# zlib-ng/minizip-ng

Measured on NVIDIA H100. Metric: deflate_l1_crc32_input_throughput, higher is better.
Workload: dtype u8

## Files before the change

minizip-ng_b200/csrc/deflate_kernel.cuh:

```cuda
#ifndef MZ_DEFLATE_KERNEL_CUH
#define MZ_DEFLATE_KERNEL_CUH

#include "mzcuda_common.cuh"

namespace mzc {

constexpr int DF_THREADS = 512;
constexpr int DF_WARPS = DF_THREADS / 32;
constexpr int DF_CHUNK_MAX = 65536;
constexpr int DF_UNIT = 32768;
constexpr int DF_SB = DF_UNIT;
constexpr int DF_SPAN = 8;
constexpr int DF_BATCH = DF_THREADS * DF_SPAN;
constexpr int DF_NBATCH = DF_UNIT / DF_BATCH;
constexpr int DF_MINMATCH = 4;
constexpr int DF_LOCKLEN = 8;
constexpr int DF_HASH_BITS = 13;
constexpr int DF_HASH_ENTRIES = 1 << DF_HASH_BITS;
constexpr int DF_STAGE_WORDS = DF_UNIT / 4 + 64;
constexpr int DF_HDR_WORDS = 96;

constexpr uint32_t DF_FLAG_FINAL = 1u;
constexpr uint32_t DF_FLAG_DICT = 2u;

constexpr int DF_OFF_IN = 0;
constexpr int DF_OFF_HASH = DF_OFF_IN + DF_UNIT + 64;
constexpr int DF_OFF_STAGE = DF_OFF_HASH;
constexpr int DF_OFF_REC = DF_OFF_HASH + DF_STAGE_WORDS * 4;
constexpr int DF_OFF_SPN = DF_OFF_REC + DF_NBATCH * DF_THREADS * 8;
constexpr int DF_SPAN_BYTES = DF_NBATCH * DF_THREADS * 10;
constexpr int DF_OFF_HIST = DF_OFF_REC + DF_SPAN_BYTES;
constexpr int DF_OFF_HIST2 = DF_OFF_HIST + (288 + 32) * 4;
constexpr int DF_OFF_CODE = DF_OFF_HIST2 + 256 * 4;
constexpr int DF_OFF_LENS = DF_OFF_CODE + (288 + 32) * 4;
constexpr int DF_OFF_BITS = DF_OFF_LENS + (288 + 32);
constexpr int DF_OFF_SCAN = DF_OFF_BITS + (288 + 32);
constexpr int DF_OFF_BB = DF_OFF_SCAN + 256 * 4;
constexpr int DF_OFF_MISC = DF_OFF_BB + 512 * 4;
constexpr int DF_OFF_SINK = DF_OFF_MISC + 32 * 4 + 16;
constexpr int DF_OFF_LSYM = DF_OFF_SINK + 32 * 4;
constexpr int DF_SMEM_BYTES = DF_OFF_LSYM + 256 * 2;
constexpr uint32_t DF_ZERO_SYM = 286;
static_assert(DF_HASH_ENTRIES * 4 <= DF_STAGE_WORDS * 4, "hash fits the staging region");
constexpr int DFH_PREV = 32768;
constexpr int DFH_HASH_BITS = 14;
constexpr int DFH_OFF_HASH = (DF_SMEM_BYTES + 15) & ~15;
constexpr int DFH_SMEM_BYTES = DFH_PREV + DFH_OFF_HASH + (4 << DFH_HASH_BITS);
static_assert(DFH_SMEM_BYTES <= 227 * 1024, "shared memory budget of the history variant");
static_assert(DF_SMEM_BYTES <= 113 * 1024, "shared memory budget for two CTAs per SM");

enum { MISC_CHUNK = 3, MISC_CARRY = 8  };

struct DeflateParams {
    const uint8_t *in;
    const uint64_t *in_off;
    const uint32_t *in_len;
    const uint8_t *flags;
    uint64_t total_len;
    uint32_t chunk_size;
    uint32_t nchunks;
    uint32_t last_flags;
    int32_t level;
    uint8_t *out;
    uint64_t slot_stride;
    uint32_t *out_len;
    uint32_t *work_counter;
};

__host__ __device__ inline uint64_t deflate_slot_bound(uint32_t chunk_size) {
    return (((uint64_t)chunk_size + 12ull * ((chunk_size + DF_SB - 1) / DF_SB + 1) + 64 + 15) & ~15ull);
}

__device__ __forceinline__ void length_symbol(uint32_t len, uint32_t &sym, uint32_t &ebits, uint32_t &eval) {
    const uint32_t l = len - 3;
    const uint32_t msb = 31u - (uint32_t)__clz((int)(l | 4u));
    uint32_t e = msb - 2;
    uint32_t sy = 4 * (e + 1) + ((l >> e) & 3u);
    uint32_t ev = l & ((1u << e) - 1u);
    sy = l < 8 ? l : sy;
    const bool top = len == 258;
    sym = top ? 28u : sy;
    ebits = top ? 0u : e;
    eval = top ? 0u : ev;
}
__device__ __forceinline__ void dist_symbol0(uint32_t d, uint32_t &sym, uint32_t &ebits) {
    uint32_t m = 31u - (uint32_t)__clz((int)(d | 1u));
    ebits = m > 0 ? m - 1 : 0u;
    sym = 2 * m + ((d >> ebits) & 1u);
}
__device__ __forceinline__ uint32_t len_extra_bits(uint32_t lsym) { return (lsym < 8 || lsym >= 28) ? 0u : (lsym >> 2) - 1; }
__device__ __forceinline__ uint32_t dist_extra_bits(uint32_t dsym) { return dsym < 4 ? 0u : (dsym >> 1) - 1; }

__device__ __forceinline__ uint32_t stage_word(uint32_t base, uint32_t pos, uint32_t k4) { return base + __umulhi(pos, 1u << 27) * k4; }

__device__ __forceinline__ void stage_put(uint32_t *stage, uint32_t pos, uint32_t v, uint32_t n) {
    if (n == 0) return;
    if (n < 32) v &= (1u << n) - 1;
    uint32_t w = pos >> 5, s = pos & 31;
    atomicOr(&stage[w], v << s);
    if (s + n > 32) atomicOr(&stage[w + 1], v >> (32 - s));
}

__device__ __forceinline__ void stage_or(const Smem &sm, uint32_t pos, uint32_t v, uint32_t n) {
    const uint32_t sh = pos & 31u, wa = DF_OFF_STAGE + ((pos >> 5) << 2);
    sm.red_or32(wa, v << sh);
    if (sh + n > 32) sm.red_or32(wa + 4, v >> (32 - sh));
}

struct BitWriter {
    Smem sm;
    uint64_t acc;
    uint32_t nb, wa;
    __device__ __forceinline__ void init(const Smem &s, uint32_t bitoff) {
        sm = s; wa = DF_OFF_STAGE + (bitoff >> 5) * 4; nb = bitoff & 31; acc = 0;
    }
    __device__ __forceinline__ void put(uint32_t v, uint32_t n) {
        acc |= (uint64_t)v << nb;
        nb += n;
        if (nb >= 32) {
            sm.red_or32(wa, (uint32_t)acc);
            acc >>= 32; nb -= 32; wa += 4;
        }
    }
    __device__ __forceinline__ uint32_t bitpos() const { return ((wa - (uint32_t)DF_OFF_STAGE) << 3) + nb; }
    __device__ __forceinline__ void finish() {
        if (nb > 0) sm.red_or32(wa, (uint32_t)acc);
        if (nb > 32) sm.red_or32(wa + 4, (uint32_t)(acc >> 32));
    }
};

__device__ inline uint32_t block_excl_sum(uint32_t v, uint32_t *scan, uint32_t &total) {
    uint32_t incl = warp_incl_sum(v);
    if (lane_id() == 31) scan[warp_id()] = incl;
    __syncthreads();
    if (warp_id() == 0) {
        uint32_t w = lane_id() < (unsigned)DF_WARPS ? scan[lane_id()] : 0u;
        uint32_t wi = warp_incl_sum(w);
        scan[32 + lane_id()] = wi - w;
        if (lane_id() == 31) scan[31] = wi;
    }
    __syncthreads();
    uint32_t res = scan[32 + warp_id()] + incl - v;
    total = scan[31];
    __syncthreads();
    return res;
}

constexpr int DF_BB_THREADS = 320;
enum { BB_STAT = 0 , BB_KRAFT = 8 , BB_K = 72 ,
       BB_NEXT = 104 , BB_SLACK = 136 , BB_CNTW = 144 ,
       BB_NZ = 464 , BB_ST = 474 ,
       BB_HSUM = 484 , BB_HDRBITS = 494  };

constexpr uint64_t CL_LENS = 0x12ddad91b725bb4ull;
constexpr uint64_t CL_CODE_LO = 0x840013930ef3c6ull, CL_CODE_HI = 0xd5c7fdf6cb149ull;
constexpr uint64_t CL_ORDER57 = 0x1b6d6db248db92dull;
__device__ __forceinline__ uint32_t cl_len(uint32_t s) { return (uint32_t)(CL_LENS >> (3 * s)) & 7u; }
__device__ __forceinline__ uint32_t cl_code(uint32_t s) {
    return s < 10 ? (uint32_t)(CL_CODE_LO >> (6 * s)) & 63u : (uint32_t)(CL_CODE_HI >> (6 * (s - 10))) & 63u;
}

__device__ __forceinline__ void bb_count_lengths(uint32_t *cntw_row, uint32_t L, unsigned lane, unsigned &m) {
    if (lane < 16) cntw_row[lane] = 0;
    __syncwarp();
    m = __match_any_sync(MZ_FULL_MASK, L);
    if (L > 0 && lane == (unsigned)(__ffs((int)m) - 1)) cntw_row[L] = (uint32_t)__popc(m);
    __syncwarp();
}

__device__ inline void block_build_codes(const uint32_t *hist_ll, const uint32_t *hist_lit2, const uint32_t *hist_d, uint8_t *lens_ll, uint8_t *lens_d,
                                         uint32_t *code_ll, uint32_t *code_d, uint8_t *bits_ll, uint8_t *bits_d, uint32_t *bb,
                                         uint32_t *stage, uint32_t hdrpos, uint32_t bfinal) {
    const uint32_t tid = threadIdx.x;
    const unsigned lane = lane_id(), w = warp_id();
    const int a = tid < 288 ? 0 : (tid < 320 ? 1 : 2);
    const uint32_t sym = a == 0 ? tid : tid - 288;
    const uint32_t nsym = a == 0 ? 286u : 30u;
    const int M = 15;
    const uint32_t one = 1u << M;
    const uint32_t w0 = a == 0 ? 0u : 9u;
    uint32_t c = (a < 2 && sym < nsym) ? (a == 0 ? hist_ll[sym] + (sym < 256 ? hist_lit2[sym] : 0u) : hist_d[sym]) : 0u;

    if (tid < 144) bb[tid] = (tid == BB_STAT + 2 || tid == BB_STAT + 6) ? 0xffffffffu : 0u;
    bar_sync(1, DF_BB_THREADS);
    if (a < 2) {
        uint32_t used_w = __reduce_add_sync(MZ_FULL_MASK, c ? 1u : 0u);
        uint32_t tot_w = __reduce_add_sync(MZ_FULL_MASK, c);
        uint32_t first_w = __reduce_min_sync(MZ_FULL_MASK, c ? sym : 0xffffffffu);
        if (lane == 0) {
            atomicAdd(&bb[BB_STAT + a * 4 + 0], used_w);
            atomicAdd(&bb[BB_STAT + a * 4 + 1], tot_w);
            atomicMin(&bb[BB_STAT + a * 4 + 2], first_w);
        }
    }
    bar_sync(1, DF_BB_THREADS);
    float ideal = 0.f;
    if (a < 2) {
        uint32_t used = bb[BB_STAT + a * 4 + 0], total = bb[BB_STAT + a * 4 + 1], fu = bb[BB_STAT + a * 4 + 2];
        if (used < 2) {
            uint32_t d0 = used == 0 ? 0u : (fu == 0 ? 1u : 0u);
            uint32_t d1 = used == 0 ? 1u : d0;
            if ((sym == d0 || sym == d1) && c == 0) c = 1;
            total += 2 - used;
        }
        if (c) ideal = __log2f((float)total) - __log2f((float)c);
    }
    float lo = -3.0f, step = 0.25f;
    uint32_t slack[2] = {0, 0};
    for (int sweep = 0; sweep < 2; sweep++) {
        if (a < 2) {
#pragma unroll
            for (int cnd = 0; cnd < 16; cnd++) {
                uint32_t kr = 0;
                if (c) {
                    int l = (int)ceilf(ideal - (lo + step * (float)cnd));
                    l = l < 1 ? 1 : (l > M ? M : l);
                    kr = 1u << (M - l);
                }
                kr = __reduce_add_sync(MZ_FULL_MASK, kr);
                if (lane == 0) atomicAdd(&bb[BB_KRAFT + sweep * 32 + a * 16 + cnd], kr);
            }
        }
        bar_sync(1, DF_BB_THREADS);
        float lo_a = lo;
        for (int aa = 0; aa < 2; aa++) {
            int best = 0;
            for (int cnd = 1; cnd < 16; cnd++)
                if (bb[BB_KRAFT + sweep * 32 + aa * 16 + cnd] <= one) best = cnd;
            slack[aa] = one - bb[BB_KRAFT + sweep * 32 + aa * 16 + best];
            if (aa == a) lo_a = lo + step * (float)best;
        }
        lo = lo_a;
        step *= 0.0625f;
    }
    uint32_t L = 0;
    if (c) {
        int l = (int)ceilf(ideal - lo);
        L = (uint32_t)(l < 1 ? 1 : (l > M ? M : l));
    }
    unsigned m = 0;
    int buf = 0;
    for (int pass = 0; pass < 40; pass++) {
        if (slack[0] == 0 && slack[1] == 0) break;
        uint32_t *cntw = bb + BB_CNTW + buf * 160;
        if (a < 2) bb_count_lengths(cntw + w * 16, L, lane, m);
        bar_sync(1, DF_BB_THREADS);
        if (w == 0 || w == 9) {
            const int aa = w == 0 ? 0 : 1;
            const uint32_t wa = aa == 0 ? 0u : 9u, wb = aa == 0 ? 9u : 10u;
            uint32_t tot = 0;
            if (lane >= 2 && lane <= (unsigned)M)
                for (uint32_t ww = wa; ww < wb; ww++) tot += cntw[ww * 16 + lane];
            uint32_t sl = slack[aa], myk = 0;
            for (int len = 2; len <= M; len++) {
                uint32_t t = __shfl_sync(MZ_FULL_MASK, tot, len);
                uint32_t can = sl >> (M - len);
                uint32_t k = t < can ? t : can;
                if (lane == (unsigned)len) myk = k;
                sl -= k << (M - len);
            }
            if (lane >= 2 && lane <= (unsigned)M) bb[BB_K + aa * 16 + lane] = myk;
            if (lane == 0) bb[BB_SLACK + aa] = sl;
        }
        bar_sync(1, DF_BB_THREADS);
        if (a < 2 && L >= 2) {
            uint32_t rank = (uint32_t)__popc(m & ((1u << lane) - 1));
            for (uint32_t ww = w0; ww < w; ww++) rank += cntw[ww * 16 + L];
            if (rank < bb[BB_K + a * 16 + L]) L -= 1;
        }
        slack[0] = bb[BB_SLACK + 0];
        slack[1] = bb[BB_SLACK + 1];
        buf ^= 1;
    }
    uint32_t *cntw = bb + BB_CNTW + buf * 160;
    if (a < 2) bb_count_lengths(cntw + w * 16, L, lane, m);
    bar_sync(1, DF_BB_THREADS);
    if (w == 0 || w == 9) {
        const int aa = w == 0 ? 0 : 1;
        const uint32_t wa = aa == 0 ? 0u : 9u, wb = aa == 0 ? 9u : 10u;
        uint32_t tot = 0;
        if (lane >= 1 && lane <= (unsigned)M)
            for (uint32_t ww = wa; ww < wb; ww++) tot += cntw[ww * 16 + lane];
        uint32_t code = 0, prev = 0, mycode = 0;
        for (int len = 1; len <= M; len++) {
            code = (code + prev) << 1;
            if (lane == (unsigned)len) mycode = code;
            prev = __shfl_sync(MZ_FULL_MASK, tot, len);
        }
        if (lane >= 1 && lane <= (unsigned)M) bb[BB_NEXT + aa * 16 + lane] = mycode;
    }
    bar_sync(1, DF_BB_THREADS);
    if (a < 2) {
        uint32_t cw = 0;
        if (L) {
            uint32_t rank = (uint32_t)__popc(m & ((1u << lane) - 1));
            for (uint32_t ww = w0; ww < w; ww++) rank += cntw[ww * 16 + L];
            uint32_t code = bb[BB_NEXT + a * 16 + L] + rank;
            cw = (__brev(code) >> (32 - L)) | (L << 16);
        }
        if (a == 0) {
            const uint32_t eb = sym >= 257 ? len_extra_bits(sym - 257) : 0u;
            lens_ll[sym] = (uint8_t)L;
            code_ll[sym] = cw | (eb << 20);
            bits_ll[sym] = (uint8_t)(L + eb);
        } else {
            lens_d[sym] = (uint8_t)L;
            code_d[sym] = cw;
            bits_d[sym] = (uint8_t)(L + dist_extra_bits(sym));
        }
    }
    const unsigned nz = __ballot_sync(MZ_FULL_MASK, L != 0);
    if (lane == 0) bb[BB_NZ + w] = nz;
    bar_sync(1, DF_BB_THREADS);
    const uint32_t hlit = 256u + 32u - (uint32_t)__clz((int)bb[BB_NZ + 8]);
    const uint32_t hdw = bb[BB_NZ + 9];
    const uint32_t hdist = hdw ? 32u - (uint32_t)__clz((int)hdw) : 1u;
    const uint32_t nlen = a == 0 ? hlit : hdist;
    const bool valid = sym < nlen;
    const uint32_t prevL = sym == 0 ? 0xffu : (a == 0 ? lens_ll[sym - 1] : lens_d[sym - 1]);
    const unsigned st = __ballot_sync(MZ_FULL_MASK, (valid && prevL != L) || sym == nlen);
    if (lane == 0) bb[BB_ST + w] = st;
    bar_sync(1, DF_BB_THREADS);
    uint32_t nb = 0, val = 0;
    if (valid) {
        uint32_t m = st & (0xffffffffu >> (31u - lane)), ww = w;
        while (m == 0) m = bb[BB_ST + --ww];
        const uint32_t s0 = (ww - w0) * 32u + 31u - (uint32_t)__clz((int)m);
        m = lane == 31 ? 0u : st & (0xfffffffeu << lane);
        ww = w;
        while (m == 0) m = bb[BB_ST + ++ww];
        const uint32_t e0 = (ww - w0) * 32u + (uint32_t)__ffs((int)m) - 1u;
        const uint32_t k = sym - s0, R = e0 - s0;
        uint32_t cs = L, ev = 0, eb = 0;
        bool tok = true;
        if (L == 0) {
            const uint32_t full = (R / 138u) * 138u, rem = R - full;
            if (k < full) { tok = k % 138u == 0; cs = 18; ev = 127; eb = 7; }
            else if (rem >= 11) { tok = k == full; cs = 18; ev = rem - 11; eb = 7; }
            else if (rem >= 3) { tok = k == full; cs = 17; ev = rem - 3; eb = 3; }
        } else if (k > 0) {
            const uint32_t k1 = k - 1, rest = R - 1, full = (rest / 6u) * 6u, rem = rest - full;
            if (k1 < full) { tok = k1 % 6u == 0; cs = 16; ev = 3; eb = 2; }
            else if (rem >= 3) { tok = k1 == full; cs = 16; ev = rem - 3; eb = 2; }
        }
        if (tok) {
            const uint32_t cl = cl_len(cs);
            nb = cl + eb;
            val = cl_code(cs) | (ev << cl);
        }
    }
    const uint32_t incl = warp_incl_sum(nb);
    if (lane == 31) bb[BB_HSUM + w] = incl;
    bar_sync(1, DF_BB_THREADS);
    uint32_t off = incl - nb, total = 0;
    for (uint32_t ww = 0; ww < 10; ww++) {
        const uint32_t t = bb[BB_HSUM + ww];
        off += ww < w ? t : 0u;
        total += t;
    }
    if (nb) stage_put(stage, hdrpos + 17 + 57 + off, val, nb);
    if (tid == 0) {
        stage_put(stage, hdrpos, bfinal | (2u << 1) | ((hlit - 257u) << 3) | ((hdist - 1u) << 8) | (15u << 13), 17);
        bb[BB_HDRBITS] = 17 + 57 + total;
    }
    if (tid == 32) stage_put(stage, hdrpos + 17, (uint32_t)CL_ORDER57, 32);
    if (tid == 64) stage_put(stage, hdrpos + 17 + 32, (uint32_t)(CL_ORDER57 >> 32), 25);
}

__device__ __forceinline__ uint32_t extend_match8(const Smem &sm, uint32_t c, uint32_t q, uint32_t maxlen) {
    uint32_t len = 8;
    while (len < maxlen) {
        uint32_t x = sm.ld32u(DF_OFF_IN, q + len) ^ sm.ld32u(DF_OFF_IN, c + len);
        if (x) {
            len += (uint32_t)(__ffs((int)x) - 1) >> 3;
            break;
        }
        len += 4;
    }
    return len < maxlen ? len : maxlen;
}

__device__ __forceinline__ uint32_t opaque4() { return blockDim.x / (uint32_t)(DF_THREADS / 4); }

template <bool HIST>
__device__ __forceinline__ uint32_t hash_addr(uint32_t v, uint32_t k4) {
    return (HIST ? DFH_OFF_HASH : DF_OFF_HASH) + __umulhi(v * 2654435761u, 1u << (HIST ? DFH_HASH_BITS : DF_HASH_BITS)) * k4;
}

__device__ __forceinline__ uint32_t rec_len(uint32_t r) { uint32_t l = (r >> 3) & 255u; return l ? l + 3 : 0u; }

__device__ __forceinline__ uint32_t fin_len(uint32_t m) { return ((m >> 4) & 255u) + 3u; }
__device__ __forceinline__ uint32_t fin_dist(uint32_t m) { return ((m >> 12) & 0x7fffu) + 1u; }
template <bool ONEM>
__device__ __forceinline__ void span_classify(const Smem &sm, uint32_t A, uint32_t B, uint32_t q0, uint32_t cover, uint32_t &F, uint32_t &MA,
                                              uint32_t &MB) {
    const uint32_t lit = (A >> 26) | ((B >> 26) << 6);
    const uint32_t crel = cover > q0 ? cover - q0 : 0u;
    const uint32_t cr8 = crel < 8 ? crel : 8u;
    uint32_t ex = 0;
    MA = MB = 0;
#pragma unroll
    for (int r = 0; r < (ONEM ? 1 : 2); r++) {
        const uint32_t R = r == 0 ? A : B;
        const uint32_t j = R & 7u, end = j + rec_len(R);
        const uint32_t s = j > crel ? j : crel;
        const uint32_t Lf = (end > s ? end : s) - s;
        const uint32_t P = (s < 8u ? s : 8u) & 7u;
        const uint32_t M = Lf >= 3 ? (((Lf << 4) + (0x80000000u - (3u << 4))) | P | ((R << 1) & (0x7fffu << 12))) : 0u;
        if (r == 0) MA = M;
        else MB = M;
        ex = Lf - 1u < 2u ? Lf : ex;
    }
    F = ((lit >> cr8) << cr8) | (ex << 8);
    if (ex) {
        const uint32_t p = DF_OFF_IN + q0 + crel;
        F |= sm.ld8(p) << 16;
        if (ex == 2) F |= sm.ld8(p + 1) << 24;
    }
}

__device__ __forceinline__ uint32_t match_symbols(const Smem &sm, uint32_t M) {
    uint32_t ds, db;
    const uint32_t lsv = sm.ld16(DF_OFF_LSYM + ((M >> 3) & 0x1feu));
    const uint32_t d = fin_dist(M) - 1;
    dist_symbol0(d, ds, db);
    sm.red_add32(DF_OFF_HIST + (257u + (lsv & 31u)) * 4, 1u);
    sm.red_add32(DF_OFF_HIST + (288u + ds) * 4, 1u);
    return 0x80000000u | ((M & 7u) << 28) | ((d & ((1u << db) - 1u)) << 15) | (ds << 10) | lsv;
}
__device__ __forceinline__ uint32_t match_bits(const Smem &sm, uint32_t M) {
    const uint32_t n = sm.ld8(DF_OFF_BITS + 257u + (M & 31u)) + sm.ld8(DF_OFF_BITS + 288u + ((M >> 10) & 31u));
    return M ? n : 0u;
}
__device__ __forceinline__ void put_match_bits(const Smem &sm, uint32_t pos, uint32_t M) {
    const uint32_t cwl = sm.ld32(DF_OFF_CODE + (257u + (M & 31u)) * 4);
    const uint32_t cwd = sm.ld32(DF_OFF_CODE + (288u + ((M >> 10) & 31u)) * 4);
    const uint32_t cl = (cwl >> 16) & 15u, cd = (cwd >> 16) & 15u;
    const uint32_t v1 = (cwl & 0x7fffu) | (((M >> 5) & 31u) << cl);
    const uint32_t n1 = cl + ((cwl >> 20) & 15u);
    const uint32_t v2 = (cwd & 0x7fffu) | (((M >> 15) & 0x1fffu) << cd);
    const uint64_t V = (uint64_t)v1 | ((uint64_t)v2 << n1);
    const uint32_t lo = (uint32_t)V, hi = (uint32_t)(V >> 32);
    const uint32_t wa = stage_word(DF_OFF_STAGE, pos, opaque4());
    const uint32_t w0 = __funnelshift_l(0u, lo, pos), w1 = __funnelshift_l(lo, hi, pos), w2 = __funnelshift_l(hi, 0u, pos);
    sm.red_or32(wa, w0);
    sm.red_or32(wa + 4, w1);
    if (w2) sm.red_or32(wa + 8, w2);
}

__device__ __forceinline__ uint32_t nth_parked(const uint32_t (&bm)[DF_NBATCH], uint32_t k, uint32_t warp) {
    uint32_t r = k, word = 0, bsel = 0;
    bool found = false;
#pragma unroll
    for (int b = 0; b < DF_NBATCH; b++) {
        const uint32_t c = (uint32_t)__popc(bm[b]);
        const bool here = !found && r < c;
        word = here ? bm[b] : word;
        bsel = here ? (uint32_t)b : bsel;
        found = found || here;
        r -= found ? 0u : c;
    }
    uint32_t base = 0;
#pragma unroll
    for (int st = 16; st; st >>= 1) {
        const uint32_t c = (uint32_t)__popc((word >> base) & ((1u << st) - 1u));
        const bool up = r >= c;
        r -= up ? c : 0u;
        base += up ? (uint32_t)st : 0u;
    }
    return found ? bsel * (uint32_t)DF_THREADS + warp * 32u + base : 0xffffffffu;
}

enum { DF_PH_LOAD, DF_PH_PARSE, DF_PH_M0, DF_PH_COVER, DF_PH_T_M1, DF_PH_D, DF_PH_E_SCAN, DF_PH_F_M3, DF_PH_FLUSH, DF_PH_UNITS, DF_PH_COLS };
constexpr int DF_PH_ROWS = 1024;
#if defined(MZ_DF_PHASES) && !defined(MZ_EMU)
__device__ unsigned long long g_df_phases[DF_PH_ROWS][DF_PH_COLS];
#define DF_PHASE_BEGIN(t) unsigned long long t = clock64()
#define DF_PHASE(t, ph)                                                                        \
    do {                                                                                       \
        if (threadIdx.x == 0 && blockIdx.x < (unsigned)DF_PH_ROWS) {                           \
            const unsigned long long now_ = clock64();                                         \
            atomicAdd(&g_df_phases[blockIdx.x][ph], now_ - (t));                               \
            if ((ph) == DF_PH_LOAD) atomicAdd(&g_df_phases[blockIdx.x][DF_PH_UNITS], 1ull);   \
            (t) = now_;                                                                        \
        }                                                                                      \
    } while (0)
#else
#define DF_PHASE_BEGIN(t)
#define DF_PHASE(t, ph)
#endif

template <int STRIDE, bool LAZY, bool HIST = false>
__global__ void __launch_bounds__(DF_THREADS, HIST ? 1 : 2) deflate_chunks_kernel(DeflateParams P) {
    MZ_DYN_SMEM(smem_raw);
    uint8_t *const smem = smem_raw + (HIST ? DFH_PREV : 0);
    constexpr uint32_t CUR = HIST ? (uint32_t)DFH_PREV : 0u;
    uint8_t *s_in = smem + DF_OFF_IN;
    uint32_t *s_stage = (uint32_t *)(smem + DF_OFF_STAGE);
    uint32_t *s_hist_ll = (uint32_t *)(smem + DF_OFF_HIST);
    uint32_t *s_hist_d = s_hist_ll + 288;
    uint32_t *s_code_ll = (uint32_t *)(smem + DF_OFF_CODE);
    uint32_t *s_code_d = s_code_ll + 288;
    uint8_t *s_lens_ll = smem + DF_OFF_LENS;
    uint8_t *s_lens_d = s_lens_ll + 288;
    uint8_t *s_bits_ll = smem + DF_OFF_BITS;
    uint8_t *s_bits_d = s_bits_ll + 288;
    uint32_t *s_scan = (uint32_t *)(smem + DF_OFF_SCAN);
    uint32_t *s_bb = (uint32_t *)(smem + DF_OFF_BB);
    uint32_t *s_misc = (uint32_t *)(smem + DF_OFF_MISC);
#ifndef MZ_EMU
    uint64_t *s_bar = (uint64_t *)(smem + DF_OFF_MISC + 32 * 4);
    uint32_t bar_phase = 0;
    if (threadIdx.x == 0) {
        mbar_init(s_bar, 1);
        mbar_fence_init();
    }
    __syncthreads();
#endif
    const uint32_t tid = threadIdx.x;
    const unsigned lane = lane_id(), warp = warp_id();
    Smem sm;
    sm.init(smem);
    if (tid < 256) {
        uint32_t ls, lb, lv;
        length_symbol(tid + 3, ls, lb, lv);
        sm.st16(DF_OFF_LSYM + tid * 2, ls | (lv << 5));
    }
    constexpr bool ONEM = false;
    DF_PHASE_BEGIN(ph_t);

    for (uint32_t chunk_static = blockIdx.x;; chunk_static += gridDim.x) {
        uint32_t chunk = chunk_static;
        if (P.work_counter) {
            if (tid == 0) s_misc[MISC_CHUNK] = atomicAdd(P.work_counter, 1u);
            __syncthreads();
            chunk = s_misc[MISC_CHUNK];
        }
        if (chunk >= P.nchunks) {
            if (P.work_counter && tid == 0 && atomicAdd(P.work_counter + 1, 1u) == gridDim.x - 1) {
                P.work_counter[0] = 0;
                P.work_counter[1] = 0;
            }
            break;
        }
        uint64_t off;
        uint32_t len, flags;
        if (P.in_off) {
            off = P.in_off[chunk];
            len = P.in_len[chunk];
            flags = P.flags ? P.flags[chunk] : 0u;
        } else {
            off = (uint64_t)chunk * P.chunk_size;
            uint64_t rem = P.total_len - off;
            len = rem < P.chunk_size ? (uint32_t)rem : P.chunk_size;
            flags = P.flags ? P.flags[chunk] : ((chunk == P.nchunks - 1 ? P.last_flags & ~DF_FLAG_DICT : 0u) | (P.last_flags & DF_FLAG_DICT));
        }
        const bool dict = HIST && (flags & DF_FLAG_DICT) && off >= (uint64_t)DFH_PREV;
        uint8_t *gout = P.out + (uint64_t)chunk * P.slot_stride;

        uint32_t flushed = 0;
        uint32_t bitpos = 0;
        const uint32_t nunits = (len + DF_UNIT - 1) / DF_UNIT;
        if (tid < 4) s_misc[MISC_CARRY + tid] = 0;

        if (len == 0) {
            for (uint32_t i = tid; i < 64; i += DF_THREADS) s_stage[i] = 0;
            __syncthreads();
            if (flags & DF_FLAG_FINAL) {
                if (tid == 0) stage_put(s_stage, 0, 1u | (1u << 1), 3);
                bitpos = 10;
            }
            __syncthreads();
        }

        for (uint32_t u = 0; u < nunits; u++) {
            const uint32_t ustart = u * DF_UNIT;
            const uint32_t ulen = (ustart + DF_UNIT < len) ? (uint32_t)DF_UNIT : len - ustart;
            const uint8_t *gin = P.in + off + ustart;
            const bool last_unit = u == nunits - 1;
            const uint32_t nb = (ulen + DF_BATCH - 1) / DF_BATCH;

            const uint32_t len16 = ulen & ~15u;
            bool bulk = false;
#ifndef MZ_EMU
            bulk = (((uintptr_t)gin) & 15) == 0 && len16 > 0;
            if (bulk && tid == 0) {
                fence_proxy_async();
                mbar_expect_tx(s_bar, len16);
                tma_load_1d(s_in, gin, len16, s_bar);
            }
#endif
            if (!bulk) {
                if ((((uintptr_t)gin) & 15) == 0) {
                    for (uint32_t i = tid * 16; i < len16; i += DF_THREADS * 16) *(uint4 *)(s_in + i) = ldg_stream((const uint4 *)(gin + i));
                } else {
                    for (uint32_t i = tid; i < len16; i += DF_THREADS) s_in[i] = gin[i];
                }
            }
            for (uint32_t i = len16 + tid; i < ulen; i += DF_THREADS) s_in[i] = gin[i];
            for (uint32_t i = ulen + tid; i < ((ulen + 63) & ~15u) + 16 && i < DF_UNIT + 64; i += DF_THREADS) s_in[i] = 0;
            if (P.level != 0) {
                if (!HIST) {
                    for (uint32_t i = tid; i < DF_HASH_ENTRIES / 4; i += DF_THREADS) sm.st128(DF_OFF_HASH + i * 16, ~0u, ~0u, ~0u, ~0u);
                } else if (u == 0) {
                    for (uint32_t i = tid; i < (1u << DFH_HASH_BITS) / 4; i += DF_THREADS) sm.st128(DFH_OFF_HASH + i * 16, ~0u, ~0u, ~0u, ~0u);
                    if (dict) {
                        const uint8_t *gp = P.in + off - DFH_PREV;
                        if ((((uintptr_t)gp) & 15) == 0) {
                            for (uint32_t i = tid * 16; i < (uint32_t)DFH_PREV; i += DF_THREADS * 16) *(uint4 *)(smem - DFH_PREV + i) = ldg_stream((const uint4 *)(gp + i));
                        } else {
                            for (uint32_t i = tid; i < (uint32_t)DFH_PREV; i += DF_THREADS) smem[(int)i - DFH_PREV] = gp[i];
                        }
                    }
                } else {
                    for (uint32_t i = tid; i < (1u << DFH_HASH_BITS) / 4; i += DF_THREADS) {
                        uint4 e = *(const uint4 *)(smem + DFH_OFF_HASH + i * 16);
                        e.x = (e.x != ~0u && (e.x & 0xffffu) >= (uint32_t)DFH_PREV) ? e.x + 0x78000u : ~0u;
                        e.y = (e.y != ~0u && (e.y & 0xffffu) >= (uint32_t)DFH_PREV) ? e.y + 0x78000u : ~0u;
                        e.z = (e.z != ~0u && (e.z & 0xffffu) >= (uint32_t)DFH_PREV) ? e.z + 0x78000u : ~0u;
                        e.w = (e.w != ~0u && (e.w & 0xffffu) >= (uint32_t)DFH_PREV) ? e.w + 0x78000u : ~0u;
                        *(uint4 *)(smem + DFH_OFF_HASH + i * 16) = e;
                    }
                }
            }
#ifndef MZ_EMU
            if (bulk) {
                mbar_wait(s_bar, bar_phase);
                bar_phase ^= 1;
            }
#endif
            __syncthreads();
            if (HIST && P.level != 0 && u == 0 && dict) {
#pragma unroll 1
                for (uint32_t b = 0; b < (uint32_t)DF_NBATCH; b++) {
                    const uint32_t p0 = b * DF_BATCH + tid * DF_SPAN;
                    const uint2 x = sm.ld64((uint32_t)(DF_OFF_IN - DFH_PREV) + p0);
                    const uint32_t y = sm.ld32((uint32_t)(DF_OFF_IN - DFH_PREV) + p0 + 8);
                    const uint32_t key0 = ((15u - b) << 16) | p0;
#pragma unroll
                    for (int j = 0; j < 8; j++) {
                        const uint32_t v = j == 0 ? x.x : (j < 4 ? __funnelshift_r(x.x, x.y, 8 * j) : (j == 4 ? x.y : __funnelshift_r(x.y, y, 8 * (j - 4))));
                        sm.red_min32(hash_addr<true>(v, 4u), key0 + j);
                    }
                }
                __syncthreads();
            }
            DF_PHASE(ph_t, DF_PH_LOAD);

            uint32_t fF[DF_NBATCH], fA[DF_NBATCH];
            bool stored = (P.level == 0);
            const uint32_t bfinal = (last_unit && (flags & DF_FLAG_FINAL)) ? 1u : 0u;
            uint32_t tokbits = 0;

            if (P.level != 0) {
#pragma unroll 1
                for (uint32_t b = 0; b < nb; b++) {
                    const uint32_t q0 = b * DF_BATCH + tid * DF_SPAN;
                    uint32_t v[12], ha[8], lc[8];
                    const uint32_t k4 = opaque4();
                    {
                        const uint2 x = sm.ld64(DF_OFF_IN + q0), y = sm.ld64(DF_OFF_IN + q0 + 8);
                        v[0] = x.x; v[4] = x.y; v[8] = y.x;
#pragma unroll
                        for (int k = 1; k < 4; k++) {
                            v[k] = __funnelshift_r(x.x, x.y, 8 * k);
                            v[4 + k] = __funnelshift_r(x.y, y.x, 8 * k);
                            v[8 + k] = __funnelshift_r(y.x, y.y, 8 * k);
                        }
                    }
#pragma unroll
                    for (int j = 0; j < 8; j++) {
                        ha[j] = hash_addr<HIST>(v[j], k4);
                        if (j % STRIDE == 0) lc[j] = sm.ld32(ha[j]);
                    }
                    const uint32_t nvalid = ulen > q0 ? (ulen - q0 < 8 ? ulen - q0 : 8u) : 0u;
                    __syncthreads();
                    {
                        const uint32_t key0 = ((uint32_t)(DF_NBATCH - 1 - b) << 16) | (CUR + q0);
#pragma unroll
                        for (int j = 0; j < 8; j++) sm.red_min32(ha[j], key0 + j);
                    }
                    __syncthreads();
#pragma unroll
                    for (int j = 0; j < 8; j++) {
                        if (j % STRIDE != 0) {
                            lc[j] = 0;
                            continue;
                        }
                        const uint32_t cn = sm.ld32(ha[j]) & 0xffffu;
                        const uint32_t pq = CUR + q0 + j;
                        const uint32_t c = cn < pq ? cn : (lc[j] & 0xffffu);
                        const uint32_t ca = DF_OFF_IN - CUR + (c & ~3u);
                        const uint32_t w0 = sm.ld32(ca), w1 = sm.ld32(ca + 4), w2 = sm.ld32(ca + 8);
                        const uint32_t s = c << 3;
                        const uint32_t x0 = __funnelshift_r(w0, w1, s) ^ v[j];
                        const uint32_t x1 = __funnelshift_r(w1, w2, s) ^ v[j + 4];
                        const bool reach = c < pq && (!HIST || c >= q0 + j);
                        const uint32_t l = (reach && x0 == 0) ? 4u + ((uint32_t)__clz((int)__brev(x1)) >> 3) : 0u;
                        lc[j] = l | ((pq - c - 1u) << 4);
                    }
                    if (q0 + 16 > ulen) {
#pragma unroll
                        for (int j = 0; j < 8; j += STRIDE) {
                            const uint32_t room = ulen > q0 + j ? ulen - (q0 + j) : 0u;
                            uint32_t l = lc[j] & 15u;
                            l = l < room ? l : room;
                            lc[j] = (lc[j] & ~15u) | (l >= (uint32_t)DF_MINMATCH ? l : 0u);
                        }
                    }
                    uint32_t nxt = 0, lit = 0, mA = 0, mB = 0, span_end = 0;
                    if (STRIDE == 2 && !LAZY && !ONEM) {
                        uint32_t endA = 0, endB = 0;
#pragma unroll
                        for (int j = 6; j >= 0; j -= 2) {
                            const uint32_t l = lc[j] & 15u;
                            const uint32_t rec = (uint32_t)j | ((l - 3) << 3) | ((lc[j] >> 4) << 11);
                            mA = l ? rec : mA;
                            endA = l ? (uint32_t)j + l : endA;
                        }
#pragma unroll
                        for (int j = 6; j >= 2; j -= 2) {
                            const uint32_t l = lc[j] & 15u;
                            const uint32_t rec = (uint32_t)j | ((l - 3) << 3) | ((lc[j] >> 4) << 11);
                            const bool nextm = l != 0 && (uint32_t)j >= endA;
                            mB = nextm ? rec : mB;
                            endB = nextm ? (uint32_t)j + l : endB;
                        }
                        lit = ~(((1u << endA) - (1u << (mA & 7u))) | ((1u << endB) - (1u << (mB & 7u)))) & 0xffu;
                        span_end = mB ? endB : endA;
                    } else {
#pragma unroll
                        for (int j = 0; j < 8; j++) {
                            const bool take = nxt == (uint32_t)j;
                            if (j % STRIDE == 0) {
                                const uint32_t l = lc[j] & 15u;
                                bool ism = take && l >= (uint32_t)DF_MINMATCH;
                                if (LAZY && STRIDE == 1 && j < 7) ism = ism && !((lc[j + 1] & 15u) > l);
                                const uint32_t rec = (uint32_t)j | ((l - 3) << 3) | ((lc[j] >> 4) << 11);
                                const bool first = mA == 0;
                                if (ONEM) ism = ism && first;
                                mA = (ism && first) ? rec : mA;
                                if (!ONEM) mB = (ism && !first) ? rec : mB;
                                lit |= (take && !ism) ? (1u << j) : 0u;
                                nxt = ism ? (uint32_t)j + l : (take ? (uint32_t)j + 1u : nxt);
                            } else {
                                lit |= take ? (1u << j) : 0u;
                                nxt = take ? (uint32_t)j + 1u : nxt;
                            }
                        }
                        const uint32_t last = mB ? mB : mA;
                        span_end = last ? (last & 7u) + rec_len(last) : 0u;
                    }
                    lit &= (1u << nvalid) - 1u;
                    {
                        const uint32_t last = mB ? mB : mA;
                        const uint32_t capped = __ballot_sync(MZ_FULL_MASK, ((last >> 3) & 255u) == (uint32_t)(DF_LOCKLEN - 3));
                        if (lane == 0) s_scan[b * DF_WARPS + warp] = capped;
                        sm.st64(DF_OFF_REC + (b * DF_THREADS + tid) * 8, mA | ((lit & 63u) << 26), mB | ((lit >> 6) << 26));
                        sm.st16(DF_OFF_SPN + (b * DF_THREADS + tid) * 2, ((last & 7u) << 9) | span_end);
                    }
                }
                DF_PHASE(ph_t, DF_PH_PARSE);
                {
                    __syncwarp();
                    uint32_t bmX[DF_NBATCH], totX = 0;
#pragma unroll
                    for (int b = 0; b < DF_NBATCH; b++) {
                        bmX[b] = (uint32_t)b < nb ? s_scan[b * DF_WARPS + warp] : 0u;
                        totX += (uint32_t)__popc(bmX[b]);
                    }
                    for (uint32_t k0 = 0; k0 < totX; k0 += 32) {
                        const uint32_t sidx = nth_parked(bmX, k0 + lane, warp);
                        if (sidx != 0xffffffffu) {
                            const uint2 r = sm.ld64(DF_OFF_REC + sidx * 8);
                            const bool second = (r.y & 0x03ffffffu) != 0;
                            const uint32_t w = second ? r.y : r.x, last = w & 0x03ffffffu;
                            const uint32_t j = last & 7u, q = sidx * DF_SPAN + j, c = q - ((last >> 11) & 0x7fffu) - 1u;
                            uint32_t maxlen = ulen - q;
                            maxlen = maxlen < 258 ? maxlen : 258u;
                            uint32_t l = 0, cb = c;
                            if (q >= 4) {
                                const uint32_t a0 = sm.ld32u(DF_OFF_IN, q), a1 = sm.ld32u(DF_OFF_IN, q + 4);
                                const bool p4 = a0 == a1, p3 = __funnelshift_r(a0, a1, 24) == a0;
                                if (p4 || p3) {
                                    uint32_t cn = c;
                                    if (p4) {
                                        if (a0 == sm.ld32u(DF_OFF_IN, q - 4)) cn = q - 4;
                                        if (a0 == sm.ld32u(DF_OFF_IN, q - 2)) cn = q - 2;
                                        if (a0 == sm.ld32u(DF_OFF_IN, q - 1)) cn = q - 1;
                                    } else if (a0 == sm.ld32u(DF_OFF_IN, q - 3) && a1 == sm.ld32u(DF_OFF_IN, q + 1)) {
                                        cn = q - 3;
                                    }
                                    if (cn != c) {
// ... 322 lines not shown
```

Baseline: 141.0.

## Restructure Huffman code builder to cut barriers and shared atomics

Rewrites block_build_codes so per-warp statistics and Kraft sums are written to per-warp slots and reduced with warp shuffles/ballots rather than shared atomics. The length-adjust loop now computes canonical code bases and each symbol's rank inside the same pass, which removes the separate final count/code pass and its barriers. Run-boundary lookup for the header now uses ballot/shuffle instead of serial loops, and the previous-length read uses shuffles. It also adds optional phase-timing counters; the change carries risk of subtle rank or canonical-code errors in edge cases.

```diff
diff --git a/minizip-ng_b200/csrc/deflate_kernel.cuh b/minizip-ng_b200/csrc/deflate_kernel.cuh
--- a/minizip-ng_b200/csrc/deflate_kernel.cuh
+++ b/minizip-ng_b200/csrc/deflate_kernel.cuh
@@ -146,11 +146,37 @@
     return res;
 }
 
+enum { DF_PH_LOAD, DF_PH_PARSE, DF_PH_M0, DF_PH_COVER, DF_PH_T_M1, DF_PH_D, DF_PH_E_SCAN, DF_PH_F_M3, DF_PH_FLUSH, DF_PH_UNITS,
+       DF_PH_D_STATS, DF_PH_D_SWEEP0, DF_PH_D_SWEEP1, DF_PH_D_CODES, DF_PH_D_PASSES, DF_PH_COLS = DF_PH_D_PASSES + 4 };
+constexpr int DF_PH_ROWS = 1024;
+#if defined(MZ_DF_PHASES) && !defined(MZ_EMU)
+__device__ unsigned long long g_df_phases[DF_PH_ROWS][DF_PH_COLS];
+#define DF_PHASE_BEGIN(t) unsigned long long t = clock64()
+#define DF_PHASE(t, ph)                                                                        \
+    do {                                                                                       \
+        if (threadIdx.x == 0 && blockIdx.x < (unsigned)DF_PH_ROWS) {                           \
+            const unsigned long long now_ = clock64();                                         \
+            atomicAdd(&g_df_phases[blockIdx.x][ph], now_ - (t));                               \
+            if ((ph) == DF_PH_LOAD) atomicAdd(&g_df_phases[blockIdx.x][DF_PH_UNITS], 1ull);   \
+            (t) = now_;                                                                        \
+        }                                                                                      \
+    } while (0)
+#define DF_PHASE_COUNT(col)                                                                    \
+    do {                                                                                       \
+        if (threadIdx.x == 0 && blockIdx.x < (unsigned)DF_PH_ROWS) atomicAdd(&g_df_phases[blockIdx.x][col], 1ull); \
+    } while (0)
+#else
+#define DF_PHASE_BEGIN(t)
+#define DF_PHASE(t, ph)
+#define DF_PHASE_COUNT(col)
+#endif
+
 constexpr int DF_BB_THREADS = 320;
-enum { BB_STAT = 0 , BB_KRAFT = 8 , BB_K = 72 ,
-       BB_NEXT = 104 , BB_SLACK = 136 , BB_CNTW = 144 ,
-       BB_NZ = 464 , BB_ST = 474 ,
-       BB_HSUM = 484 , BB_HDRBITS = 494  };
+enum { BB_SW = 0 , BB_CNTW = 0 ,
+       BB_HDRBITS = 0 , BB_STW = 320 ,
+       BB_P = 320 , BB_KN = 448 ,
+       BB_SLACK = 480 , BB_NZ = 482 , BB_ST = 492 , BB_HSUM = 502  };
+static_assert(BB_HSUM + 10 <= 512, "code-builder scratch");
 
 constexpr uint64_t CL_LENS = 0x12ddad91b725bb4ull;
 constexpr uint64_t CL_CODE_LO = 0x840013930ef3c6ull, CL_CODE_HI = 0xd5c7fdf6cb149ull;
@@ -160,15 +186,7 @@
     return s < 10 ? (uint32_t)(CL_CODE_LO >> (6 * s)) & 63u : (uint32_t)(CL_CODE_HI >> (6 * (s - 10))) & 63u;
 }
 
-__device__ __forceinline__ void bb_count_lengths(uint32_t *cntw_row, uint32_t L, unsigned lane, unsigned &m) {
-    if (lane < 16) cntw_row[lane] = 0;
-    __syncwarp();
-    m = __match_any_sync(MZ_FULL_MASK, L);
-    if (L > 0 && lane == (unsigned)(__ffs((int)m) - 1)) cntw_row[L] = (uint32_t)__popc(m);
-    __syncwarp();
-}
-
-__device__ inline void block_build_codes(const uint32_t *hist_ll, const uint32_t *hist_lit2, const uint32_t *hist_d, uint8_t *lens_ll, uint8_t *lens_d,
+__device__ inline int block_build_codes(const uint32_t *hist_ll, const uint32_t *hist_lit2, const uint32_t *hist_d, uint8_t *lens_ll, uint8_t *lens_d,
                                          uint32_t *code_ll, uint32_t *code_d, uint8_t *bits_ll, uint8_t *bits_d, uint32_t *bb,
                                          uint32_t *stage, uint32_t hdrpos, uint32_t bfinal) {
     const uint32_t tid = threadIdx.x;
@@ -180,23 +198,23 @@
     const uint32_t one = 1u << M;
     const uint32_t w0 = a == 0 ? 0u : 9u;
     uint32_t c = (a < 2 && sym < nsym) ? (a == 0 ? hist_ll[sym] + (sym < 256 ? hist_lit2[sym] : 0u) : hist_d[sym]) : 0u;
-
-    if (tid < 144) bb[tid] = (tid == BB_STAT + 2 || tid == BB_STAT + 6) ? 0xffffffffu : 0u;
+    DF_PHASE_BEGIN(ph_d);
+
+    {
+        const uint32_t used_w = __reduce_add_sync(MZ_FULL_MASK, c ? 1u : 0u);
+        const uint32_t tot_w = __reduce_add_sync(MZ_FULL_MASK, c);
+        const uint32_t first_w = __reduce_min_sync(MZ_FULL_MASK, c ? sym : 0xffffffffu);
+        if (lane < 3) bb[BB_STW + w * 3 + lane] = lane == 0 ? used_w : (lane == 1 ? tot_w : first_w);
+    }
     bar_sync(1, DF_BB_THREADS);
-    if (a < 2) {
-        uint32_t used_w = __reduce_add_sync(MZ_FULL_MASK, c ? 1u : 0u);
-        uint32_t tot_w = __reduce_add_sync(MZ_FULL_MASK, c);
-        uint32_t first_w = __reduce_min_sync(MZ_FULL_MASK, c ? sym : 0xffffffffu);
-        if (lane == 0) {
-            atomicAdd(&bb[BB_STAT + a * 4 + 0], used_w);
-            atomicAdd(&bb[BB_STAT + a * 4 + 1], tot_w);
-            atomicMin(&bb[BB_STAT + a * 4 + 2], first_w);
-        }
-    }
-    bar_sync(1, DF_BB_THREADS);
+    DF_PHASE(ph_d, DF_PH_D_STATS);
     float ideal = 0.f;
     if (a < 2) {
-        uint32_t used = bb[BB_STAT + a * 4 + 0], total = bb[BB_STAT + a * 4 + 1], fu = bb[BB_STAT + a * 4 + 2];
+        const bool row = lane < (a == 0 ? 9u : 1u);
+        const uint32_t *st = bb + BB_STW + (w0 + lane) * 3;
+        uint32_t used = __reduce_add_sync(MZ_FULL_MASK, row ? st[0] : 0u);
+        uint32_t total = __reduce_add_sync(MZ_FULL_MASK, row ? st[1] : 0u);
+        const uint32_t fu = __reduce_min_sync(MZ_FULL_MASK, row ? st[2] : 0xffffffffu);
         if (used < 2) {
             uint32_t d0 = used == 0 ? 0u : (fu == 0 ? 1u : 0u);
             uint32_t d1 = used == 0 ? 1u : d0;
@@ -208,7 +226,9 @@
     float lo = -3.0f, step = 0.25f;
     uint32_t slack[2] = {0, 0};
     for (int sweep = 0; sweep < 2; sweep++) {
-        if (a < 2) {
+        uint32_t *sw = bb + BB_SW + sweep * 160;
+        {
+            uint32_t mine = 0;
 #pragma unroll
             for (int cnd = 0; cnd < 16; cnd++) {
                 uint32_t kr = 0;
@@ -218,19 +238,25 @@
                     kr = 1u << (M - l);
                 }
                 kr = __reduce_add_sync(MZ_FULL_MASK, kr);
-                if (lane == 0) atomicAdd(&bb[BB_KRAFT + sweep * 32 + a * 16 + cnd], kr);
-            }
+                mine = lane == (unsigned)cnd ? kr : mine;
+            }
+            if (lane < 16) sw[w * 16 + lane] = mine;
         }
         bar_sync(1, DF_BB_THREADS);
-        float lo_a = lo;
-        for (int aa = 0; aa < 2; aa++) {
-            int best = 0;
-            for (int cnd = 1; cnd < 16; cnd++)
-                if (bb[BB_KRAFT + sweep * 32 + aa * 16 + cnd] <= one) best = cnd;
-            slack[aa] = one - bb[BB_KRAFT + sweep * 32 + aa * 16 + best];
-            if (aa == a) lo_a = lo + step * (float)best;
-        }
-        lo = lo_a;
+        DF_PHASE(ph_d, DF_PH_D_SWEEP0 + sweep);
+        {
+            const uint32_t aa = lane >> 4, cnd = lane & 15u;
+            uint32_t kr = 0;
+#pragma unroll
+            for (uint32_t j = 0; j < 9; j++)
+                if (aa == 0 || j == 0) kr += sw[((aa ? 9u : 0u) + j) * 16 + cnd];
+            const unsigned ok = __ballot_sync(MZ_FULL_MASK, cnd > 0 && kr <= one);
+            const uint32_t ok0 = ok & 0xffffu, ok1 = ok >> 16;
+            const uint32_t best0 = ok0 ? 31u - (uint32_t)__clz((int)ok0) : 0u, best1 = ok1 ? 31u - (uint32_t)__clz((int)ok1) : 0u;
+            slack[0] = one - __shfl_sync(MZ_FULL_MASK, kr, best0);
+            slack[1] = one - __shfl_sync(MZ_FULL_MASK, kr, 16 + best1);
+            lo = lo + step * (float)(a == 0 ? best0 : best1);
+        }
         step *= 0.0625f;
     }
     uint32_t L = 0;
@@ -238,19 +264,35 @@
         int l = (int)ceilf(ideal - lo);
         L = (uint32_t)(l < 1 ? 1 : (l > M ? M : l));
     }
-    unsigned m = 0;
-    int buf = 0;
-    for (int pass = 0; pass < 40; pass++) {
-        if (slack[0] == 0 && slack[1] == 0) break;
-        uint32_t *cntw = bb + BB_CNTW + buf * 160;
-        if (a < 2) bb_count_lengths(cntw + w * 16, L, lane, m);
+    {
+        const unsigned nz = __ballot_sync(MZ_FULL_MASK, L != 0);
+        if (lane == 0) bb[BB_NZ + w] = nz;
+    }
+    const bool slack0 = slack[0] != 0 || slack[1] != 0;
+    const unsigned lt = (1u << lane) - 1u;
+    uint32_t code = 0, prev_last = 0;
+    int pass = 0;
+    for (;;) {
+        uint32_t *mk = bb + BB_CNTW + (pass & 1) * 160;
+        if (lane < 16) mk[w * 16 + lane] = 0;
+        __syncwarp();
+        const unsigned m = __match_any_sync(MZ_FULL_MASK, L);
+        if (L > 0 && (m & lt) == 0) mk[w * 16 + L] = m;
+        if (lane == 31) mk[w * 16] = L;
         bar_sync(1, DF_BB_THREADS);
         if (w == 0 || w == 9) {
             const int aa = w == 0 ? 0 : 1;
-            const uint32_t wa = aa == 0 ? 0u : 9u, wb = aa == 0 ? 9u : 10u;
             uint32_t tot = 0;
-            if (lane >= 2 && lane <= (unsigned)M)
-                for (uint32_t ww = wa; ww < wb; ww++) tot += cntw[ww * 16 + lane];
+            if (aa == 0) {
+#pragma unroll
+                for (uint32_t ww = 0; ww < 9; ww++) {
+                    if (ww > 0 && lane < 16) bb[BB_P + (ww - 1) * 16 + lane] = tot;
+                    tot += (uint32_t)__popc(mk[ww * 16 + (lane & 15u)]);
+                }
+            } else {
+                tot = (uint32_t)__popc(mk[9 * 16 + (lane & 15u)]);
+            }
+            tot = lane >= 1 && lane <= (unsigned)M ? tot : 0u;
             uint32_t sl = slack[aa], myk = 0;
             for (int len = 2; len <= M; len++) {
                 uint32_t t = __shfl_sync(MZ_FULL_MASK, tot, len);
@@ -259,45 +301,49 @@
                 if (lane == (unsigned)len) myk = k;
                 sl -= k << (M - len);
             }
-            if (lane >= 2 && lane <= (unsigned)M) bb[BB_K + aa * 16 + lane] = myk;
+            const uint32_t cnt = tot - myk + __shfl_down_sync(MZ_FULL_MASK, myk, 1);
+            const bool coded = lane >= 1 && lane <= (unsigned)M;
+            const uint32_t wgt = coded ? cnt << (M - lane) : 0u;
+            const uint32_t below = warp_incl_sum(wgt) - wgt;
+            const uint32_t mycode = coded ? below >> (M - lane) : 0u;
+            if (coded) bb[BB_KN + aa * 16 + lane] = mycode | (myk << 16);
             if (lane == 0) bb[BB_SLACK + aa] = sl;
         }
         bar_sync(1, DF_BB_THREADS);
-        if (a < 2 && L >= 2) {
-            uint32_t rank = (uint32_t)__popc(m & ((1u << lane) - 1));
-            for (uint32_t ww = w0; ww < w; ww++) rank += cntw[ww * 16 + L];
-            if (rank < bb[BB_K + a * 16 + L]) L -= 1;
+        if (a < 2 && L) {
+            const uint32_t *pw = bb + BB_P + (w - 1) * 16;
+            const bool first_w = w == w0;
+            const uint32_t rl = (first_w ? 0u : pw[L]) + (uint32_t)__popc(m & lt), kl = bb[BB_KN + a * 16 + L] >> 16;
+            const bool sh = rl < kl;
+            const uint32_t x = sh ? L - 1 : L + 1;
+            uint32_t rx = 0, kx = 0;
+            if (x >= 1 && x <= (uint32_t)M) {
+                rx = (first_w ? 0u : pw[x]) + (uint32_t)__popc(mk[w * 16 + x] & lt);
+                kx = bb[BB_KN + a * 16 + x] >> 16;
+            }
+            L -= sh ? 1u : 0u;
+            const uint32_t rank = sh ? rx - (rx < kx ? rx : kx) + rl : rl - kl + (rx < kx ? rx : kx);
+            code = (bb[BB_KN + a * 16 + L] & 0xffffu) + rank;
+        }
+        if (lane == 0 && w != w0) {
+            const uint32_t *mp = mk + (w - 1) * 16;
+            const uint32_t lp = mp[0];
+            prev_last = lp;
+            if (lp) {
+                const uint32_t rp = (w - 1 == w0 ? 0u : bb[BB_P + (w - 2) * 16 + lp]) + (uint32_t)__popc(mp[lp] & 0x7fffffffu);
+                prev_last = lp - (rp < (bb[BB_KN + a * 16 + lp] >> 16) ? 1u : 0u);
+            }
         }
         slack[0] = bb[BB_SLACK + 0];
         slack[1] = bb[BB_SLACK + 1];
-        buf ^= 1;
-    }
-    uint32_t *cntw = bb + BB_CNTW + buf * 160;
-    if (a < 2) bb_count_lengths(cntw + w * 16, L, lane, m);
-    bar_sync(1, DF_BB_THREADS);
-    if (w == 0 || w == 9) {
-        const int aa = w == 0 ? 0 : 1;
-        const uint32_t wa = aa == 0 ? 0u : 9u, wb = aa == 0 ? 9u : 10u;
-        uint32_t tot = 0;
-        if (lane >= 1 && lane <= (unsigned)M)
-            for (uint32_t ww = wa; ww < wb; ww++) tot += cntw[ww * 16 + lane];
-        uint32_t code = 0, prev = 0, mycode = 0;
-        for (int len = 1; len <= M; len++) {
-            code = (code + prev) << 1;
-            if (lane == (unsigned)len) mycode = code;
-            prev = __shfl_sync(MZ_FULL_MASK, tot, len);
-        }
-        if (lane >= 1 && lane <= (unsigned)M) bb[BB_NEXT + aa * 16 + lane] = mycode;
-    }
-    bar_sync(1, DF_BB_THREADS);
+        pass++;
+        if ((slack[0] == 0 && slack[1] == 0) || pass == 40) break;
+    }
+    if (!slack0) pass = 0;
+    DF_PHASE(ph_d, DF_PH_D_CODES);
+    DF_PHASE_COUNT(DF_PH_D_PASSES + (pass < 3 ? pass : 3));
     if (a < 2) {
-        uint32_t cw = 0;
-        if (L) {
-            uint32_t rank = (uint32_t)__popc(m & ((1u << lane) - 1));
-            for (uint32_t ww = w0; ww < w; ww++) rank += cntw[ww * 16 + L];
-            uint32_t code = bb[BB_NEXT + a * 16 + L] + rank;
-            cw = (__brev(code) >> (32 - L)) | (L << 16);
-        }
+        const uint32_t cw = L ? (__brev(code) >> (32 - L)) | (L << 16) : 0u;
         if (a == 0) {
             const uint32_t eb = sym >= 257 ? len_extra_bits(sym - 257) : 0u;
             lens_ll[sym] = (uint8_t)L;
@@ -309,26 +355,29 @@
             bits_d[sym] = (uint8_t)(L + dist_extra_bits(sym));
         }
     }
-    const unsigned nz = __ballot_sync(MZ_FULL_MASK, L != 0);
-    if (lane == 0) bb[BB_NZ + w] = nz;
-    bar_sync(1, DF_BB_THREADS);
     const uint32_t hlit = 256u + 32u - (uint32_t)__clz((int)bb[BB_NZ + 8]);
     const uint32_t hdw = bb[BB_NZ + 9];
     const uint32_t hdist = hdw ? 32u - (uint32_t)__clz((int)hdw) : 1u;
     const uint32_t nlen = a == 0 ? hlit : hdist;
     const bool valid = sym < nlen;
-    const uint32_t prevL = sym == 0 ? 0xffu : (a == 0 ? lens_ll[sym - 1] : lens_d[sym - 1]);
+    const uint32_t up = __shfl_up_sync(MZ_FULL_MASK, L, 1);
+    const uint32_t prevL = sym == 0 ? 0xffu : (lane == 0 ? prev_last : up);
     const unsigned st = __ballot_sync(MZ_FULL_MASK, (valid && prevL != L) || sym == nlen);
     if (lane == 0) bb[BB_ST + w] = st;
     bar_sync(1, DF_BB_THREADS);
+    const uint32_t stj = lane < 10u ? bb[BB_ST + lane] : 0u;
+    const unsigned stw = __ballot_sync(MZ_FULL_MASK, stj != 0);
+    const unsigned below = stw & ((1u << w) - 1u), above = stw & ~((2u << w) - 1u);
+    const uint32_t wbelow = below ? 31u - (uint32_t)__clz((int)below) : w, wabove = above ? (uint32_t)__ffs((int)above) - 1u : w;
+    const uint32_t stbelow = __shfl_sync(MZ_FULL_MASK, stj, wbelow), stabove = __shfl_sync(MZ_FULL_MASK, stj, wabove);
     uint32_t nb = 0, val = 0;
     if (valid) {
         uint32_t m = st & (0xffffffffu >> (31u - lane)), ww = w;
-        while (m == 0) m = bb[BB_ST + --ww];
+        if (m == 0) { m = stbelow; ww = wbelow; }
         const uint32_t s0 = (ww - w0) * 32u + 31u - (uint32_t)__clz((int)m);
         m = lane == 31 ? 0u : st & (0xfffffffeu << lane);
         ww = w;
-        while (m == 0) m = bb[BB_ST + ++ww];
+        if (m == 0) { m = stabove; ww = wabove; }
         const uint32_t e0 = (ww - w0) * 32u + (uint32_t)__ffs((int)m) - 1u;
         const uint32_t k = sym - s0, R = e0 - s0;
         uint32_t cs = L, ev = 0, eb = 0;
@@ -365,6 +414,7 @@
     }
     if (tid == 32) stage_put(stage, hdrpos + 17, (uint32_t)CL_ORDER57, 32);
     if (tid == 64) stage_put(stage, hdrpos + 17 + 32, (uint32_t)(CL_ORDER57 >> 32), 25);
+    return pass;
 }
 
 __device__ __forceinline__ uint32_t extend_match8(const Smem &sm, uint32_t c, uint32_t q, uint32_t maxlen) {
@@ -470,25 +520,6 @@
     }
     return found ? bsel * (uint32_t)DF_THREADS + warp * 32u + base : 0xffffffffu;
 }
-
-enum { DF_PH_LOAD, DF_PH_PARSE, DF_PH_M0, DF_PH_COVER, DF_PH_T_M1, DF_PH_D, DF_PH_E_SCAN, DF_PH_F_M3, DF_PH_FLUSH, DF_PH_UNITS, DF_PH_COLS };
-constexpr int DF_PH_ROWS = 1024;
-#if defined(MZ_DF_PHASES) && !defined(MZ_EMU)
-__device__ unsigned long long g_df_phases[DF_PH_ROWS][DF_PH_COLS];
-#define DF_PHASE_BEGIN(t) unsigned long long t = clock64()
-#define DF_PHASE(t, ph)                                                                        \
-    do {                                                                                       \
-        if (threadIdx.x == 0 && blockIdx.x < (unsigned)DF_PH_ROWS) {                           \
-            const unsigned long long now_ = clock64();                                         \
-            atomicAdd(&g_df_phases[blockIdx.x][ph], now_ - (t));                               \
-            if ((ph) == DF_PH_LOAD) atomicAdd(&g_df_phases[blockIdx.x][DF_PH_UNITS], 1ull);   \
-            (t) = now_;                                                                        \
-        }                                                                                      \
-    } while (0)
-#else
-#define DF_PHASE_BEGIN(t)
-#define DF_PHASE(t, ph)
-#endif
 
 template <int STRIDE, bool LAZY, bool HIST = false>
 __global__ void __launch_bounds__(DF_THREADS, HIST ? 1 : 2) deflate_chunks_kernel(DeflateParams P) {
```

Result: faster. 142.8 (median of 6 runs) (+1.3%).
